# RatInABox-Lab/RatInABox

Measured on AMD Instinct MI355X. Metric: agent-steps/sec (whole node) at 4096 agents x 1024 PlaceCells, higher is better.
Workload: dtype f32 rates / f64 motion

## Files before the change

### include/riab_hip.h

```cpp
#ifndef RIAB_HIP_H
#define RIAB_HIP_H

#include <stdint.h>

#ifdef __cplusplus
extern "C" {
#endif

#define RIAB_ABI_VERSION 11
#define RIAB_MAX_WALLS 64
#define RIAB_MAX_TEST_ANGLES 360
#define RIAB_STATE_ROWS 12
#define RIAB_HIST_ROWS 8
#define RIAB_MAX_BOUNCES 16

enum {
  RIAB_OK = 0,
  RIAB_EINVAL = -1,
  RIAB_EALIGN = -2,
  RIAB_ETOOBIG = -3,
  RIAB_EUNSUPPORTED = -4,
  RIAB_EFULL = -5,
  RIAB_EPARTIAL = -6,
  RIAB_ECHANGED = -7
// ... 318 lines not shown
  RIAB_TW_EP_START = 4,
  RIAB_TW_EP_ANY_ENDED = 5,
  RIAB_TW_STARTED = 6,
  RIAB_TW_TERMINAL = 7,
  RIAB_TW_GOAL_LIST = 8,
  RIAB_TW_ROWS = 24
};
int riab_task_world_step(const RiabEnv* env, const RiabTask* task, double* task_state, double* world,
                         const double* pos_x, const double* pos_y, int64_t B, double t_env, double* reward_out,
                         uint8_t* terminal_out, uint64_t* met_scratch, int32_t* cand_scratch, int32_t* ctl,
                         int32_t* diag, riab_stream_t stream);
int riab_task_world_reset(const RiabEnv* env, const RiabTask* task, double* task_state, double* world, int64_t B,
                          int64_t agent_id0, double t_env, int32_t n_select, int32_t ordered, uint64_t seed,
                          uint64_t counter, int32_t teleport, const double* new_x, const double* new_y,
                          double* pos_x, double* pos_y, float* hist_x, float* hist_y, double* ep_log,
                          int64_t ep_log_cap, int32_t* ep_count, int32_t only_if_terminal, double gv_scale,
                          double* gv_x, double* gv_y, int32_t* diag, riab_stream_t stream);
int riab_task_world_goal_vector(const RiabEnv* env, const RiabTask* task, double* task_state, const double* world,
                                const double* pos_x, const double* pos_y, int64_t B, double scale, double* out_x,
                                double* out_y, riab_stream_t stream);

int riab_plan_set_task(RiabPlan* plan, const RiabTask* task, double* task_state, int64_t task_B, double t_env,
                       double dt_env, double* reward_out, uint8_t* terminal_out, int32_t* task_diag,
                       int32_t auto_reset, int32_t n_select, int32_t ordered, uint64_t task_seed,
                       uint64_t reset_counter, int32_t teleport, double* ep_log, int64_t ep_log_cap,
                       int32_t* ep_count, double scripted_speed);
double riab_plan_task_clock(const RiabPlan* plan);
int riab_plan_set_task_world(RiabPlan* plan, double* world, uint64_t* met_scratch, int32_t* cand_scratch, int32_t* ctl);

enum { RIAB_CTRL_STARTED = 0, RIAB_CTRL_TIMEOUTS = 1, RIAB_CTRL_ABORT = 2, RIAB_CTRL_SERIALISED = 3,
       RIAB_CTRL_STAMPS = 8,
       RIAB_CTRL_TRAJ_STAMPS = 12,
       RIAB_CTRL_PROGRESS = 32 };
#define RIAB_CTRL_PROGRESS_WORD(w) (RIAB_CTRL_PROGRESS + 32 * ((w) >> 2) + ((w) & 3))
#define RIAB_CTRL_WORDS(B) (RIAB_CTRL_PROGRESS + 32 * (((B) + 255) / 256))
enum { RIAB_TIMING_STAMPS = 0, RIAB_TIMING_EVENTS = 1 };
typedef struct RiabSimulate {
  const RiabEnv* env;
  const RiabMotion* motion;
  double* state;
  int64_t B;
  int64_t agent_id0;
  const double* drift;
  const double* noise;
  const double* forced_pos;
  const double* resample_pos;
  uint64_t seed;
  uint64_t step0;
  int32_t T;
  int32_t n_pops;
  const struct RiabPopulation* pops;
  float* hist;
  int32_t* diag;
  uint32_t* ctrl;
  int32_t timed_pop;
  int32_t timing_mode;
  const struct RiabWatch* watch;
  int32_t n_watch;
} RiabSimulate;
typedef struct RiabWatch {
  const void* live;
  const void* snapshot;
  int64_t bytes;
} RiabWatch;
typedef struct RiabStreamer RiabStreamer;
RiabStreamer* riab_streamer_create(void);
void riab_streamer_destroy(RiabStreamer* h);
enum { RIAB_STREAMER_OPT_GATE = 0, RIAB_STREAMER_OPT_POLL_MAX = 1, RIAB_STREAMER_OPT_HEAD_ROWS = 2,
       RIAB_STREAMER_OPT_SIDE_STREAM = 3, RIAB_STREAMER_OPT_STEP_NS = 4, RIAB_STREAMER_OPT_LEAD_MBPS = 5,
       RIAB_STREAMER_OPT_STRICT = 6, RIAB_STREAMER_OPT_SPIN_LIMIT = 7 };
enum { RIAB_GATE_ALWAYS = 0, RIAB_GATE_WHEN_BUSY = 1, RIAB_GATE_RESERVED = 2 };
int riab_streamer_configure(RiabStreamer* h, int32_t option, int32_t value);
int riab_streamer_warmup(RiabStreamer* h, riab_stream_t stream);
int riab_simulate(RiabStreamer* h, const RiabSimulate* run, riab_stream_t stream);
int riab_watch_compare(const RiabWatch* watch, int32_t n);
float riab_streamer_last_rate_ms(RiabStreamer* h);
enum { RIAB_FORM_NONE = 0, RIAB_FORM_ONE_KERNEL = 1, RIAB_FORM_CHUNKS = 2, RIAB_FORM_SERIAL = 3, RIAB_FORM_POPULATIONS = 4,
       RIAB_FORM_HEAD_AND_PIECES = 5 };
int riab_streamer_last_form(RiabStreamer* h);
int64_t riab_streamer_info(RiabStreamer* h, int32_t which);

enum { RIAB_OPT_TRAJ_KERNEL = 0, RIAB_OPT_FUSED_TASK = 1, RIAB_OPT_BVC_BOX = 2, RIAB_OPT_NT_STORES = 3,
       RIAB_OPT_PUB_SINGLE_ROWS = 4, RIAB_OPT_POLL_SLEEP = 5, RIAB_OPT_FUSED_STEP = 6, RIAB_OPT_STEP1_SPIN = 7,
       RIAB_OPT_STEP1_RESIDENCY = 8, RIAB_OPT_COUNT = 9 };
int riab_set_option(int32_t option, int32_t value);

int riab_host_wait_spin(int32_t on);

typedef struct RiabTDParams {
  float dt;
  float tau;
  float tau_e;
  float eta;
  float L2;
  int64_t B;
  int64_t Bp;
  int32_t n;
  int32_t Mp;
} RiabTDParams;

typedef struct RiabTDLayer {
  const float* rates;
  float* trace;
  float* wt;
  int32_t n_in;
} RiabTDLayer;

int riab_td_forward_tail(const RiabTDParams* p, const RiabTDLayer* layers, int32_t n_layers, const float* v,
                         float* v_last, float* dvdt, int32_t with_trace, riab_stream_t stream);

int64_t riab_td_workspace(const RiabTDParams* p, const RiabTDLayer* layers, int32_t n_layers);

int riab_td_update(const RiabTDParams* p, const RiabTDLayer* layers, int32_t n_layers, const void* reward,
                   int32_t reward_f64, int64_t reward_ld_n, int64_t reward_ld_b, const float* v, const float* dvdt,
                   const float* prime, float* td, int32_t fuse_trace, float* workspace, int64_t workspace_floats,
                   riab_stream_t stream);

int riab_td_reset(const RiabTDParams* p, const RiabTDLayer* layers, int32_t n_layers, float* const* rows,
                  int32_t n_rows, const uint8_t* mask, riab_stream_t stream);

int riab_td_learn_step(const RiabTDParams* p, const RiabTDLayer* layers, int32_t n_layers, const void* reward,
                       int32_t reward_f64, int64_t reward_ld_n, int64_t reward_ld_b, float* v, float* v_last, float* dvdt,
                       const float* prime, float* td, const uint8_t* mask, int32_t zero_v, float* workspace,
                       int64_t workspace_floats, riab_stream_t stream);

enum {
  RIAB_REWARD_NONE = 0,
  RIAB_REWARD_TASK = 1,
  RIAB_REWARD_POINTER = 2,
  RIAB_REWARD_POPULATION = 3
};
int riab_plan_set_learner(RiabPlan* plan, int32_t index, const RiabTDParams* p, float* const* traces, float* v_last,
                          float* dvdt, float* td, float* workspace, int64_t workspace_floats, int32_t reward_kind,
                          const void* reward, int32_t reward_f64, int64_t reward_ld_n, int64_t reward_ld_b,
                          int32_t reward_index);

enum {
  RIAB_THETA_NONE = 0,
  RIAB_THETA_BEHIND = 1,
  RIAB_THETA_AHEAD = 2
};
enum {
  RIAB_THETA_DIAG_BEHIND = 0,
  RIAB_THETA_DIAG_AHEAD = 1,
  RIAB_THETA_DIAG_ROLLOUT = 2,
  RIAB_THETA_DIAG_FAR = 3
};

int riab_theta_sequence_step(const RiabEnv* env, const double* lead_state, int64_t B, int64_t n_agents, double* ring,
                             int32_t capacity, int32_t lookback, int64_t n_records, int32_t branch, double phase, double d_half,
                             double theta_frac, const double* future, const int32_t* count, int32_t K, double* pos_out,
                             int32_t* diag, riab_stream_t stream);

int riab_theta_sequence_rollout(const RiabEnv* env, const RiabMotion* motion, const double* lead_state,
                                double* forward_state, int64_t B, int64_t n_agents, int64_t agent_id0, const double* z_in,
                                double* z_out,
                                uint64_t seed, uint64_t step0, int32_t K, double forward_distance, double* future,
                                int32_t* count, int32_t* motion_diag, int32_t* diag, riab_stream_t stream);

int riab_shift_agent_position(const double* lead_state, int64_t B, double shift_m, double* pos_out, riab_stream_t stream);

enum {
  RIAB_DUMB_DIAG_WALL_CUTS = 0,
  RIAB_DUMB_DIAG_BOUNDARY = 1,
  RIAB_DUMB_DIAG_SATURATIONS = 2
};

// ... 66 lines not shown
```

### ratinabox_amd/_lib.py

```python
import ctypes as C
import os

import torch

from . import _build

ABI_VERSION = 11
MAX_WALLS = 64
STATE_ROWS = 12
HIST_ROWS = 8

S_POS_X, S_POS_Y, S_VEL_X, S_VEL_Y, S_ROT_VEL, S_MVEL_X, S_MVEL_Y, S_MROT_VEL, S_HD_X, S_HD_Y, S_DIST, S_DWALL = range(12)
H_POS_X, H_POS_Y, H_VEL_X, H_VEL_Y, H_HD_X, H_HD_Y, H_ROT_VEL, H_DIST = range(8)

PC_DESCRIPTIONS = {"gaussian": 0, "gaussian_threshold": 1, "diff_of_gaussians": 2, "one_hot": 3, "top_hat": 4}
GEOMETRIES = {"euclidean": 0, "line_of_sight": 1, "geodesic": 2}
GC_DESCRIPTIONS = {"rectified_cosines": 0, "shifted_cosines": 1}


class RiabEnv(C.Structure):
    _fields_ = [("extent", C.c_double * 4), ("scale", C.c_double), ("periodic", C.c_int32),
                ("n_walls", C.c_int32), ("walls", C.c_void_p), ("polygon", C.c_int32), ("n_boundary", C.c_int32),
                ("hole_mask", C.c_uint64)]

# ... 235 lines not shown
    "riab_probe_compute_units": (C.c_int, [C.c_void_p, C.c_void_p]),
    "riab_plan_info": (C.c_int64, [C.c_void_p, C.c_int32]),
    "riab_task_step": (C.c_int, [C.POINTER(RiabEnv), C.POINTER(RiabTask), C.c_void_p, C.c_void_p, C.c_void_p, C.c_int64,
                                 C.c_double, C.c_void_p, C.c_void_p, C.c_void_p, C.c_void_p]),
    "riab_task_goal_vector": (C.c_int, [C.POINTER(RiabEnv), C.POINTER(RiabTask), C.c_void_p, C.c_void_p, C.c_void_p, C.c_int64,
                                        C.c_double, C.c_void_p, C.c_void_p, C.c_void_p]),
    "riab_plan_set_task": (C.c_int, [C.c_void_p, C.POINTER(RiabTask), C.c_void_p, C.c_int64, C.c_double, C.c_double,
                                     C.c_void_p, C.c_void_p, C.c_void_p, C.c_int32, C.c_int32, C.c_int32, C.c_uint64,
                                     C.c_uint64, C.c_int32, C.c_void_p, C.c_int64, C.c_void_p, C.c_double]),
    "riab_plan_task_clock": (C.c_double, [C.c_void_p]),
    "riab_task_reset": (C.c_int, [C.POINTER(RiabEnv), C.POINTER(RiabTask), C.c_void_p, C.c_void_p, C.c_int64, C.c_int64,
                                  C.c_double, C.c_int32, C.c_int32, C.c_uint64, C.c_uint64, C.c_int32, C.c_void_p,
                                  C.c_void_p, C.c_void_p, C.c_void_p, C.c_void_p, C.c_void_p, C.c_void_p, C.c_int64,
                                  C.c_void_p, C.c_void_p, C.c_void_p]),
    "riab_task_world_step": (C.c_int, [C.POINTER(RiabEnv), C.POINTER(RiabTask), C.c_void_p, C.c_void_p, C.c_void_p, C.c_void_p,
                                       C.c_int64, C.c_double, C.c_void_p, C.c_void_p, C.c_void_p, C.c_void_p, C.c_void_p,
                                       C.c_void_p, C.c_void_p]),
    "riab_task_world_reset": (C.c_int, [C.POINTER(RiabEnv), C.POINTER(RiabTask), C.c_void_p, C.c_void_p, C.c_int64, C.c_int64,
                                        C.c_double, C.c_int32, C.c_int32, C.c_uint64, C.c_uint64, C.c_int32, C.c_void_p,
                                        C.c_void_p, C.c_void_p, C.c_void_p, C.c_void_p, C.c_void_p, C.c_void_p, C.c_int64,
                                        C.c_void_p, C.c_int32, C.c_double, C.c_void_p, C.c_void_p, C.c_void_p, C.c_void_p]),
    "riab_plan_set_task_world": (C.c_int, [C.c_void_p, C.c_void_p, C.c_void_p, C.c_void_p, C.c_void_p]),
    "riab_task_world_goal_vector": (C.c_int, [C.POINTER(RiabEnv), C.POINTER(RiabTask), C.c_void_p, C.c_void_p, C.c_void_p,
                                              C.c_void_p, C.c_int64, C.c_double, C.c_void_p, C.c_void_p, C.c_void_p]),
    "riab_streamer_create": (C.c_void_p, []),
    "riab_streamer_destroy": (None, [C.c_void_p]),
    "riab_simulate": (C.c_int, [C.c_void_p, C.POINTER(RiabSimulate), C.c_void_p]),
    "riab_streamer_warmup": (C.c_int, [C.c_void_p, C.c_void_p]),
    "riab_watch_compare": (C.c_int, [C.c_void_p, C.c_int32]),
    "riab_streamer_configure": (C.c_int, [C.c_void_p, C.c_int32, C.c_int32]),
    "riab_streamer_last_rate_ms": (C.c_float, [C.c_void_p]),
    "riab_streamer_last_form": (C.c_int, [C.c_void_p]),
    "riab_streamer_info": (C.c_int64, [C.c_void_p, C.c_int32]),
    "riab_host_wait_spin": (C.c_int, [C.c_int32]),
    "riab_set_option": (C.c_int, [C.c_int32, C.c_int32]),
    "riab_abi_sizeof": (C.c_int64, [C.c_int32]),
    "riab_abi_version": (C.c_int, []),
    "riab_strerror": (C.c_char_p, [C.c_int]),
}


class RiabError(RuntimeError):
    pass


def _load():
    path = _build.LIB_PATH
    override = os.environ.get("RIAB_HIP_LIB")
    if override:
        path = override
    elif _build.is_stale():
        try:
            path = _build.build()
        except Exception as e:
            if not os.path.exists(path):
                raise ImportError(
                    "ratinabox_amd: libriab_hip.so is missing and could not be built with hipcc "
                    f"({e}). There is no CPU fallback; build it with `python -m ratinabox_amd._build`.") from e
            import warnings
            warnings.warn(f"ratinabox_amd: libriab_hip.so is older than its sources and could not be rebuilt ({e}); "
                          "loading the existing library", RuntimeWarning)
    lib = C.CDLL(path)
    for name, (res, args) in PROTOTYPES.items():
        fn = getattr(lib, name)
        fn.restype = res
        fn.argtypes = args
    if lib.riab_abi_version() != ABI_VERSION:
        raise ImportError(f"libriab_hip.so ABI {lib.riab_abi_version()} != binding ABI {ABI_VERSION}: rebuild")
    mirrors = ((0, RiabEnv), (1, RiabMotion), (2, RiabRateIO), (3, RiabPopulation), (4, RiabTask), (5, RiabFFInput),
               (7, RiabSimulate), (8, RiabWatch), (9, RiabTDParams), (10, RiabTDLayer), (11, RiabMLPLayer))
    for which, cls in mirrors:
        if lib.riab_abi_sizeof(which) != C.sizeof(cls):
            raise ImportError(f"libriab_hip.so: sizeof({cls.__name__}) is {lib.riab_abi_sizeof(which)} in the library, "
                              f"{C.sizeof(cls)} in the binding: rebuild (python -m ratinabox_amd._build --force)")
    if lib.riab_abi_sizeof(6) != TS_ROWS:
        raise ImportError(f"libriab_hip.so: RIAB_TS_ROWS is {lib.riab_abi_sizeof(6)}, the binding has {TS_ROWS}: rebuild")
    return lib, path


lib, LIB_PATH = _load()


OPTIONS = {"traj_kernel": 0, "fused_task": 1, "bvc_box": 2, "nt_stores": 3, "pub_single_rows": 4, "poll_sleep": 5,
           "fused_step": 6, "step1_spin": 7, "step1_residency": 8}


def set_option(name, value):
    old = lib.riab_set_option(OPTIONS[name], int(value))
    if old < 0:
        raise RiabError(f"riab_set_option({name}, {value}) refused")
    return old


for _name, _opt, _val in (("RIAB_NO_PC", "traj_kernel", 1), ("RIAB_TRAJ2", "traj_kernel", 2), ("RIAB_NO_FUSED_TASK", "fused_task", 0),
                          ("RIAB_NO_BVC_BOX", "bvc_box", 0), ("RIAB_NT_STORES_WIDE", "nt_stores", 1),
                          ("RIAB_NO_FUSED_STEP", "fused_step", 0), ("RIAB_FUSED_STEP_PLAIN_STORES", "fused_step", 2)):
    if os.environ.get(_name):
        set_option(_opt, _val)
for _name, _opt in (("RIAB_PUB_SINGLE_ROWS", "pub_single_rows"), ("RIAB_POLL_SLEEP", "poll_sleep"),
                    ("RIAB_STEP1_SPIN", "step1_spin"), ("RIAB_STEP1_RESIDENCY", "step1_residency")):
    if os.environ.get(_name):
        set_option(_opt, int(os.environ[_name]))


def strerror(code):
    return lib.riab_strerror(int(code)).decode()


def check(code, what):
    if code != 0:
        raise RiabError(f"{what} failed with code {code}: {strerror(code)}")


_ENV_DATA = getattr(os.environ, "_data", None)


def env(name, default=None):
    if _ENV_DATA is not None:
        v = _ENV_DATA.get(name.encode() if os.name != "nt" else name.upper())
        return default if v is None else (v.decode() if isinstance(v, bytes) else v)
    return os.environ.get(name, default)


def ptr(t):
    return None if t is None else C.c_void_p(t.data_ptr())


def current_stream():
    import torch
    raw = getattr(torch._C, "_cuda_getCurrentRawStream", None)
    if raw is not None:
        return C.c_void_p(raw(torch.cuda.current_device()))
    return C.c_void_p(torch.cuda.current_stream().cuda_stream)


_COMPUTE_UNITS = {}


def compute_units(device_index):
    n = _COMPUTE_UNITS.get(device_index)
    if n is None:
        import torch
        forced = os.environ.get("RIAB_COMPUTE_UNITS")
        if forced:
            n = int(forced)
        else:
            with torch.cuda.device(device_index):
                scratch = torch.zeros(CU_PROBE_WORDS, dtype=torch.int32, device=f"cuda:{device_index}")
                check(lib.riab_probe_compute_units(ptr(scratch), current_stream()), "riab_probe_compute_units")
                n = int(scratch[CU_PROBE_WORDS - 1].item())
            props = torch.cuda.get_device_properties(device_index).multi_processor_count
            if n < 1 or n > props:
                n = props
        _COMPUTE_UNITS[device_index] = n
    return n
```

### ratinabox_amd/csrc/riab_rates.hip

```cpp
#include <hip/hip_ext.h>

#include <type_traits>

#include "riab_device.h"
#include "riab_rate_cells.h"
#include "riab_handover.h"
#include "riab_launch.h"
#ifndef RIAB_SPIKE_POLICY_GATED
#define RIAB_SPIKE_POLICY_GATED RIAB_STORE_NT
#endif
#ifndef RIAB_SPIKE_POLICY_WIDE
#define RIAB_SPIKE_POLICY_WIDE RIAB_STORE_NT
#endif

namespace riab {


template <class Cell, int SPK, int CPB, bool NT>
__global__ __launch_bounds__(256) void rate_kernel_wide(const RateArgs a, Cell cell) {
  __shared__ double s_lds[Cell::LDS_DOUBLES];
  cell.stage(s_lds);
  constexpr int NP = Cell::NP;
  const int lane = threadIdx.x & 63;
  const int c0 = blockIdx.y * CPB;
  const uint32_t t = blockIdx.z;
  const uint32_t q = blockIdx.x * 256u + threadIdx.x;
  const bool live = q < (uint32_t)a.qrow;
  const uint32_t qc = live ? q : 0u;
  const int pi = c0 * NP + lane;
  const float mine = (lane < NP * CPB && pi < a.n * NP) ? cell.tab[pi] : 0.0f;
  const typename Cell::Pos P = cell.load(a, (int64_t)t * a.pos_ld + 4 * (int64_t)qc);
  int64_t off = ((int64_t)t * a.n + c0) * a.B + 4 * (int64_t)qc;
  const uint32_t step = a.step0 + t;
  const uint32_t group = a.group0 + qc;
  const SpikeCtx k = a.spike_ctx();
  RIAB_CELL_GROUP(Cell, CPB, cell, mine, P, c0, a.n, a.fr_scale, a.fr_min, a.rates, off, a.B, live,
                  NT ? RIAB_STORE_WT : RIAB_STORE_PLAIN, SPK == 1, SPK == 2, NT ? RIAB_STORE_WT : RIAB_SPIKE_POLICY_WIDE, k, step, group)
}

template <class Cell, int SPK>
__global__ __launch_bounds__(256) void rate_kernel_generic(const RateArgs a, Cell cell) {
  __shared__ double s_lds[Cell::LDS_DOUBLES];
  cell.stage(s_lds);
  constexpr int NP = Cell::NP;
  const uint32_t p4 = blockIdx.x * 256u + threadIdx.x;
  const bool live = p4 < a.nquads;
  const uint32_t pc = live ? p4 : 0u;
  const uint32_t t = pc / (uint32_t)a.qrow;
  const uint32_t q = pc - t * (uint32_t)a.qrow;
  const typename Cell::Pos P = cell.load(a, (int64_t)t * a.pos_ld + 4 * (int64_t)q);
  const int c0 = blockIdx.y * a.cells_per_block;
  const int c1 = min(a.n, c0 + a.cells_per_block);
  int64_t off = ((int64_t)t * a.n + c0) * a.B + 4 * (int64_t)q;
  const uint32_t step = a.step0 + t;
  const uint32_t group = a.group0 + q;
  const int lane = threadIdx.x & 63;
  for (int cb = c0; cb < c1; cb += 64) {
    float mine[NP];
    const int cm = min(cb + lane, a.n - 1);
#pragma unroll
    for (int i = 0; i < NP; ++i) mine[i] = cell.tab[cm * NP + i];
    const int cnt = min(64, c1 - cb);
    for (int j = 0; j < cnt; ++j) {
      float p[NP];
#pragma unroll
      for (int i = 0; i < NP; ++i)
        p[i] = __builtin_bit_cast(float, __builtin_amdgcn_readlane(__builtin_bit_cast(int, mine[i]), j));
      v4f r = cell.eval(p, P);
      r = finish_rate(post_scale(cell, p, P, r * a.fr_scale + a.fr_min), P);
      if (live) {
        store_stream<RIAB_STORE_NT>(a.rates + off, r);
        if (SPK == 1) spike_store<false>(a.spike_ctx(), r, off, step, (uint32_t)(cb + j), group);
        if (SPK == 2) spike_store<true>(a.spike_ctx(), r, off, step, (uint32_t)(cb + j), group);
      }
      off += a.B;
    }
  }
}

template <int GX>
__global__ __launch_bounds__(256) void place_one_hot_kernel(const RateArgs a, PlaceCell<RIAB_PC_GAUSSIAN, GX> cell) {
  __shared__ double s_lds[PlaceCell<RIAB_PC_GAUSSIAN, GX>::LDS_DOUBLES];
  cell.stage(s_lds);
  const uint32_t p4 = blockIdx.x * 256u + threadIdx.x;
  if (p4 >= a.nquads) return;
  const uint32_t t = p4 / (uint32_t)a.qrow;
  const uint32_t q = p4 - t * (uint32_t)a.qrow;
  const PosQuad P = cell.load(a, (int64_t)t * a.pos_ld + 4 * (int64_t)q);
  float best[4] = {INFINITY, INFINITY, INFINITY, INFINITY};
  int arg[4] = {0, 0, 0, 0};
// ... 86 lines not shown
    off += a.B;
  }
}

__global__ __launch_bounds__(256) void noise_kernel(float* noise, float* rates, const float* z_in, int n,
                                                    int64_t qrow, int T, float theta_dt, float sigma_dt, uint32_t k0,
                                                    uint32_t k1, uint32_t step0, uint32_t tag, uint32_t group0) {
  const int64_t q = (int64_t)blockIdx.x * 256 + threadIdx.x;
  if (q >= qrow) return;
  const int64_t row = (int64_t)n * qrow * 4;
  for (int c = blockIdx.y; c < n; c += gridDim.y) {
    const int64_t off = ((int64_t)c * qrow + q) * 4;
    v4f x = ldv4(noise + off);
    for (int t = 0; t < T; ++t) {
      v4f z;
      if (z_in) {
        z = ldv4(z_in + t * row + off);
      } else {
        const u32x4 w = philox4x32_spikes(step0 + (uint32_t)t, (uint32_t)c, group0 + (uint32_t)q, tag, k0, k1);
        const float u0 = ((float)(w.x >> 8) + 0.5f) * 0x1.0p-24f, u1 = (float)(w.y >> 8) * 0x1.0p-24f;
        const float u2 = ((float)(w.z >> 8) + 0.5f) * 0x1.0p-24f, u3 = (float)(w.w >> 8) * 0x1.0p-24f;
        const float r0 = sqrtf(-2.0f * logf(u0)), r1 = sqrtf(-2.0f * logf(u2));
        z = v4f{r0 * __builtin_amdgcn_cosf(u1), r0 * __builtin_amdgcn_sinf(u1), r1 * __builtin_amdgcn_cosf(u3),
                r1 * __builtin_amdgcn_sinf(u3)};
      }
      x = x + (-theta_dt) * x + sigma_dt * z;
      const v4f r = ldv4(rates + t * row + off);
      *reinterpret_cast<v4f*>(rates + t * row + off) = r + x;
    }
    *reinterpret_cast<v4f*>(noise + off) = x;
  }
}

__global__ __launch_bounds__(256) void fill_kernel(float* dst, int64_t n4, float value) {
  const int64_t i = (int64_t)blockIdx.x * 256 + threadIdx.x;
  if (i < n4) reinterpret_cast<v4f*>(dst)[i] = v4f{value, value, value, value};
}

struct StreamArgs {
  uint32_t* ctrl;
  uint32_t step_base;
  uint32_t spin_limit;
  uint32_t stamps;
  uint32_t sleep_max;
  uint32_t serial_rows;
  uint32_t serial_gap;
};
__device__ __forceinline__ bool ended_just_now(const uint32_t* ctrl, uint32_t gap_ticks) {
  const unsigned long long end = ld_agent(reinterpret_cast<const uint64_t*>(ctrl + RIAB_CTRL_TRAJ_STAMPS + 2));
  const unsigned long long now = __builtin_amdgcn_s_memrealtime();
  return now >= end && now - end < (unsigned long long)gap_ticks;
}
__device__ __forceinline__ int stream_progress(const StreamArgs& s, uint32_t q, int lane) {
  int rel = 0x7fffffff;
  if (lane < 4) {
    const uint32_t v = ld_agent(s.ctrl + RIAB_CTRL_PROGRESS + 32 * q + lane);
    rel = (int)(v - s.step_base);
    rel = rel < 0 ? 0 : rel;
  }
  const int r0 = __builtin_amdgcn_readlane(rel, 0), r1 = __builtin_amdgcn_readlane(rel, 1);
  const int r2 = __builtin_amdgcn_readlane(rel, 2), r3 = __builtin_amdgcn_readlane(rel, 3);
  return __builtin_amdgcn_readfirstlane(min(min(r0, r1), min(r2, r3)));
}
__device__ __forceinline__ void stream_wait(const StreamArgs& s, uint32_t q, int t, int lane) {
  int known = stream_progress(s, q, lane);
  for (uint32_t spins = 0; known <= t; ++spins) {
    const uint32_t ab = ld_agent(s.ctrl + RIAB_CTRL_ABORT);
    if (__builtin_amdgcn_readfirstlane((int)ab)) return;
    if (spins >= s.spin_limit) {
      if (lane == 0) {
        atomicAdd(s.ctrl + RIAB_CTRL_TIMEOUTS, 1u);
        st_agent(s.ctrl + RIAB_CTRL_ABORT, 1u);
      }
      return;
    }
    if (spins < 4) __builtin_amdgcn_s_sleep(4);
    else if (spins < 16 || s.sleep_max <= 16) __builtin_amdgcn_s_sleep(16);
    else if (s.sleep_max >= 48) __builtin_amdgcn_s_sleep(48);
    else __builtin_amdgcn_s_sleep(32);
    known = stream_progress(s, q, lane);
  }
}

template <class Cell, int SPK, int CPB, bool LONG, int WAVES>
__global__ __launch_bounds__(64 * WAVES) void rate_kernel_gated(const RateArgs a, Cell cell, const StreamArgs s) {
  __shared__ double s_lds[Cell::LDS_DOUBLES];
  cell.stage(s_lds);
  constexpr int NP = Cell::NP;
  static_assert(WAVES % 4 == 0, "four waves share a (1024 agents) x (CPB cells) tile");
  const int lane = threadIdx.x & 63;
  const int wv = __builtin_amdgcn_readfirstlane((int)(threadIdx.x >> 6));
  const int c0 = (int)(blockIdx.y * (WAVES / 4) + (wv >> 2)) * CPB;
  const uint32_t t = blockIdx.z;
  const uint32_t q = blockIdx.x * 256u + (threadIdx.x & 255u);
  const uint32_t wq = (uint32_t)__builtin_amdgcn_readfirstlane((int)(blockIdx.x * 4u + (uint32_t)(wv & 3)));
  if (wq * 64u >= (uint32_t)a.qrow || c0 >= a.n) return;
  const int pi = c0 * NP + lane;
  const float mine = (lane < NP * CPB && pi < a.n * NP) ? cell.tab[pi] : 0.0f;
  const bool grid_first = t == 0 && blockIdx.x == 0 && blockIdx.y == 0 && wv == 0;
  if (s.stamps && grid_first && lane == 0)
    st_agent(reinterpret_cast<uint64_t*>(s.ctrl + RIAB_CTRL_STAMPS), (uint64_t)__builtin_amdgcn_s_memrealtime());
  if (s.serial_rows >= 8u && grid_first) {
    if (stream_progress(s, wq, lane) >= (int)s.serial_rows && ended_just_now(s.ctrl, s.serial_gap) && lane == 0)
      atomicAdd(s.ctrl + RIAB_CTRL_SERIALISED, 1u);
  }
#ifdef RIAB_PIPE_PROFILE
  riab_g64* const dbg = (riab_g64*)(uintptr_t)(s.ctrl + 2048);
  const bool first_wg = blockIdx.x == 0 && blockIdx.y == 0 && threadIdx.x == 0;
  if (first_wg) dbg[1 * 64 + t] = (unsigned long long)__builtin_amdgcn_s_memrealtime();
#endif
  stream_wait(s, wq, (int)t, lane);
#ifdef RIAB_PIPE_PROFILE
  if (first_wg) dbg[2 * 64 + t] = (unsigned long long)__builtin_amdgcn_s_memrealtime();
#endif
  const int64_t po = (int64_t)t * a.pos_ld + 4 * (int64_t)q;
  const typename Cell::Pos P = cell.load_agent(a, po);
  int64_t off = ((int64_t)t * a.n + c0) * a.B + 4 * (int64_t)q;
  const uint32_t step = a.step0 + t;
  const uint32_t group = a.group0 + q;
  const SpikeCtx k = a.spike_ctx();
  RIAB_CELL_GROUP(Cell, CPB, cell, mine, P, c0, a.n, a.fr_scale, a.fr_min, a.rates, off, a.B, true, RIAB_STORE_NT, SPK == 1, false,
                  RIAB_SPIKE_POLICY_GATED, k, step, group)
#ifdef RIAB_PIPE_PROFILE
  if (c0 + CPB >= a.n && blockIdx.x + 1 == gridDim.x && (threadIdx.x & 255u) == 0) {
    drain_stores();
    dbg[3 * 64 + t] = (unsigned long long)__builtin_amdgcn_s_memrealtime();
  }
#endif
  if (s.stamps && t + 1 == gridDim.z && c0 + CPB >= a.n) {
    drain_stores();
    if (lane == 0) fetch_max_agent(reinterpret_cast<uint64_t*>(s.ctrl + RIAB_CTRL_STAMPS + 2), (uint64_t)__builtin_amdgcn_s_memrealtime());
  }
}

__global__ __launch_bounds__(64) void stream_gate_kernel(uint32_t* ctrl, uint32_t started_target, uint32_t n_traj,
                                                         uint32_t progress_target, uint32_t spin_limit, uint32_t sleep_long,
                                                         uint32_t final_target, uint32_t serial_gap) {
  const int lane = threadIdx.x;
  for (uint32_t spins = 0;; ++spins) {
    const uint32_t v = ld_agent(ctrl + RIAB_CTRL_STARTED);
    bool ok = (int32_t)(v - started_target) >= 0;
    bool all_done = ok && final_target != 0u && spins == 0u;
    if (ok) {
      for (uint32_t w = lane; w < n_traj; w += 64) {
        const uint32_t p = ld_agent(ctrl + RIAB_CTRL_PROGRESS_WORD(w));
        ok = ok && (int32_t)(p - progress_target) >= 0;
        all_done = all_done && (int32_t)(p - final_target) >= 0;
      }
    }
    if (spins == 0u && final_target != 0u && n_traj > 0u && __builtin_amdgcn_ballot_w64(!all_done) == 0 &&
        ended_just_now(ctrl, serial_gap) && lane == 0)
      atomicAdd(ctrl + RIAB_CTRL_SERIALISED, 1u);
    if (__builtin_amdgcn_ballot_w64(!ok) == 0) return;
    if (ld_agent(ctrl + RIAB_CTRL_ABORT)) return;
    if (spins >= spin_limit) {
      if (lane == 0) {
        atomicAdd(ctrl + RIAB_CTRL_TIMEOUTS, 1u);
        st_agent(ctrl + RIAB_CTRL_ABORT, 1u);
      }
      return;
    }
    if (sleep_long && spins >= 64) __builtin_amdgcn_s_sleep(127);
    else if (sleep_long) __builtin_amdgcn_s_sleep(8);
    else __builtin_amdgcn_s_sleep(16);
  }
}

__global__ __launch_bounds__(64) void stream_open_kernel(uint32_t* ctrl, uint32_t n_traj, uint32_t step_base) {
  for (uint32_t w = threadIdx.x; w < n_traj; w += 64)
    st_agent(ctrl + RIAB_CTRL_PROGRESS_WORD(w), step_base);
  if (threadIdx.x == 0)
    st_agent(ctrl + RIAB_CTRL_STARTED, 0u);
}

static int check_io(const RiabRateIO* io, int n, bool need_pos, bool need_hd) {
  if (!io || n <= 0 || io->T <= 0 || io->B <= 0 || !io->rates) return RIAB_EINVAL;
  if (need_pos && (!io->pos_x || !io->pos_y)) return RIAB_EINVAL;
  if (need_hd && (!io->hd_x || !io->hd_y)) return RIAB_EINVAL;
  if (io->B % 4 != 0 || io->pos_ld % 4 != 0 || io->agent_id0 % 4 != 0) return RIAB_EALIGN;
  const uintptr_t m = (uintptr_t)io->rates | (uintptr_t)io->pos_x | (uintptr_t)io->pos_y | (uintptr_t)io->hd_x |
                      (uintptr_t)io->hd_y | (uintptr_t)io->u_in;
  if (m & 15) return RIAB_EALIGN;
  if ((uintptr_t)io->spikes & 3) return RIAB_EALIGN;
  if (io->u_in && !io->spikes) return RIAB_EINVAL;
  if (io->T * (io->B / 4) >= ((int64_t)1 << 31)) return RIAB_ETOOBIG;
  return RIAB_OK;
}

static RateArgs make_args(const RiabRateIO* io, int n) {
  RateArgs a;
  a.pos_x = io->pos_x;
  a.pos_y = io->pos_y;
  a.hd_x = io->hd_x;
  a.hd_y = io->hd_y;
  a.pos_ld = io->pos_ld;
  a.qrow = io->B / 4;
  a.nquads = io->T * a.qrow;
  a.B = io->B;
  a.rates = io->rates;
  a.spikes = io->spikes;
  a.u_in = io->u_in;
  a.dt = io->dt;
  a.fr_scale = io->max_fr - io->min_fr;
  a.fr_min = io->min_fr;
  a.k0 = (uint32_t)io->seed;
  a.k1 = (uint32_t)(io->seed >> 32);
  a.step0 = (uint32_t)io->step0;
// ... 41 lines not shown
  if (geometry == RIAB_GEOM_EUCLIDEAN) return RIAB_OK;
  if (env->n_walls - 4 > RIAB_MAX_WALLS) return RIAB_ETOOBIG;
  if (geometry == RIAB_GEOM_GEODESIC && env->n_walls > 5) return RIAB_EUNSUPPORTED;
  return RIAB_OK;
}
static int place_geometry_check(const RiabEnv* env, int geometry) {
  if (!env->periodic && geometry != RIAB_GEOM_EUCLIDEAN && env->n_walls > 4 && !env->walls) return RIAB_EINVAL;
  return place_geometry_refused(env, geometry);
}
template <class F>
static int visit_place_geometry(const RiabEnv* env, int geometry, F&& f) {
  if (env->periodic) return f(std::integral_constant<int, 3>{});
  switch (geometry) {
    case RIAB_GEOM_EUCLIDEAN: return f(std::integral_constant<int, 0>{});
    case RIAB_GEOM_LINE_OF_SIGHT: return f(std::integral_constant<int, 1>{});
    case RIAB_GEOM_GEODESIC: return f(std::integral_constant<int, 2>{});
    default: return RIAB_EINVAL;
  }
}
template <int GX>
static int internal_walls(const RiabEnv* env) {
  const int n_internal = env->n_walls > 4 ? env->n_walls - 4 : 0;
  return (GX == 2 && n_internal > 1) ? 1 : n_internal;
}
template <int GX>
static PlaceCell<RIAB_PC_GAUSSIAN, GX> make_place_cell(const RiabEnv* env, const float* table, float top_hat_width, int n_internal) {
  return place_cell<RIAB_PC_GAUSSIAN, GX>(table, (float)env->scale, (float)(env->scale / 2), top_hat_width * top_hat_width,
                                          env->walls, n_internal, make_env_shape(env));
}
template <int GX, class F>
static int visit_place_desc(int desc, const PlaceCell<RIAB_PC_GAUSSIAN, GX>& base, int otherwise, F&& f) {
  switch (desc) {
    case RIAB_PC_GAUSSIAN: return f(base);
    case RIAB_PC_GAUSSIAN_THRESHOLD: return f(base.template as<RIAB_PC_GAUSSIAN_THRESHOLD>());
    case RIAB_PC_DIFF_OF_GAUSSIANS: return f(base.template as<RIAB_PC_DIFF_OF_GAUSSIANS>());
    case RIAB_PC_TOP_HAT: return f(base.template as<RIAB_PC_TOP_HAT>());
    default: return otherwise;
  }
}
template <class F>
static int visit_grid_desc(int desc, const float* table, float f0, F&& f) {
  if (desc == RIAB_GC_RECTIFIED) return f(GridCell<RIAB_GC_RECTIFIED>{table, f0, 1.0f / (1.0f - f0)});
  if (desc == RIAB_GC_SHIFTED) return f(GridCell<RIAB_GC_SHIFTED>{table, f0, 1.0f});
  return RIAB_EINVAL;
}

template <int GX>
static int launch_place(const RiabRateIO* io, int n, int desc, const PlaceCell<RIAB_PC_GAUSSIAN, GX>& base,
                        hipStream_t s) {
  if (desc == RIAB_PC_ONE_HOT) {
    RateArgs a = make_args(io, n);
    dim3 grid = generic_grid(&a);
    grid.y = 1;
    hipLaunchKernelGGL((place_one_hot_kernel<GX>), grid, dim3(256), 0, s, a, base);
    return (int)hipGetLastError();
  }
  return visit_place_desc(desc, base, RIAB_EINVAL, [&](const auto& c) { return launch_rate(io, n, c, s); });
}

static uint32_t serial_gap_ticks() {
  static uint32_t ticks = 0;
  if (!ticks) {
    int dev = 0, khz = 0;
    if (hipGetDevice(&dev) != hipSuccess || hipDeviceGetAttribute(&khz, hipDeviceAttributeWallClockRate, dev) != hipSuccess || khz <= 0)
      khz = 100000;
    ticks = (uint32_t)((long long)khz * 25 / 1000);
  }
  return ticks;
}

struct StreamLaunch {
  StreamArgs st;
  hipEvent_t ev0, ev1;
  int T;
  bool spikes;
  bool reserve;
  bool dry_run;
  hipStream_t s;
};

template <class Cell>
static int launch_stream_cell(const RateArgs& a, const Cell& cell, const StreamLaunch& L) {
  constexpr int CPB = (Cell::NP * 2 * Cell::CPB <= 64) ? 2 * Cell::CPB : Cell::CPB;
  using Kernel = void (*)(const RateArgs, Cell, const StreamArgs);
  static constexpr Kernel kGated[8] = {
      rate_kernel_gated<Cell, 0, CPB, false, 4>,  rate_kernel_gated<Cell, 0, CPB, true, 4>,
      rate_kernel_gated<Cell, 1, CPB, false, 4>,  rate_kernel_gated<Cell, 1, CPB, true, 4>,
      rate_kernel_gated<Cell, 0, CPB, false, 12>, rate_kernel_gated<Cell, 0, CPB, true, 12>,
      rate_kernel_gated<Cell, 1, CPB, false, 12>, rate_kernel_gated<Cell, 1, CPB, true, 12>};
  const int T = L.T;
  const int64_t groups = (a.n + CPB - 1) / CPB;
  if (T > 65535 || groups > 65535) return RIAB_ETOOBIG;
  const bool reserve = L.reserve;
  const int variant = (reserve ? 4 : 0) + (L.spikes ? 2 : 0) + (T > 256 ? 1 : 0);
  if (reserve) {
    static int regs[8] = {0, 0, 0, 0, 0, 0, 0, 0};
    int& r = regs[variant];
    if (r == 0) {
      hipFuncAttributes attr;
      const void* f = (const void*)kGated[variant];
      r = (hipFuncGetAttributes(&attr, f) == hipSuccess && attr.numRegs > 0) ? attr.numRegs : 1 << 20;
      if (r < (1 << 20) && 2 * (int64_t)attr.sharedSizeBytes + 81920 > 160 * 1024) r = 1 << 20;
      (void)hipGetLastError();
    }
    if (6 * ((r + 7) / 8 * 8) + traj_kernel_regs() > 512) return RIAB_EUNSUPPORTED;
  }
  if (L.dry_run) return RIAB_OK;
  static bool launched[8] = {false, false, false, false, false, false, false, false};
  bool& seen = launched[variant];
  StreamArgs st = L.st;
  if (!seen) st.serial_rows = 0u;
  seen = true;
  const dim3 grid((unsigned)((a.qrow + 255) / 256), (unsigned)(reserve ? (groups + 2) / 3 : groups), (unsigned)T);
  const dim3 block(reserve ? 768 : 256);
  if (L.ev0 || L.ev1) hipExtLaunchKernelGGL(kGated[variant], grid, block, 0, L.s, L.ev0, L.ev1, 0u, a, cell, st);
  else hipLaunchKernelGGL(kGated[variant], grid, block, 0, L.s, a, cell, st);
  return (int)hipGetLastError();
}

template <class F>
static int visit_stream_cell(const RiabEnv* env, const RiabPopulation* pop, F&& f) {
  switch (pop->kind) {
    case RIAB_POP_PLACE:
      return visit_place_geometry(env, pop->geometry, [&](auto gx) {
        return visit_place_desc(pop->description, make_place_cell<decltype(gx)::value>(env, pop->table, pop->top_hat_width, internal_walls<decltype(gx)::value>(env)),
                                RIAB_EUNSUPPORTED, f);
      });
    case RIAB_POP_GRID: return visit_grid_desc(pop->description, pop->table, pop->f0, f);
    case RIAB_POP_HDC: return f(HDCell<0>{pop->table, 0.0f, nullptr, nullptr});
    case RIAB_POP_PLANE_WAVE: return f(PlaneWaveCell{pop->table});
    default: return RIAB_EUNSUPPORTED;
  }
}

int stream_supported(const RiabEnv* env, const RiabPopulation* pop, int64_t B) {
  if (!env || !pop || pop->n <= 0 || B <= 0 || B % 256 != 0) return RIAB_EUNSUPPORTED;
  if (pop->noise_state) return RIAB_EUNSUPPORTED;
  switch (pop->kind) {
    case RIAB_POP_PLACE:
      if (pop->description == RIAB_PC_ONE_HOT) return RIAB_EUNSUPPORTED;
      if (place_geometry_refused(env, pop->geometry)) return RIAB_EUNSUPPORTED;
      return pop->table ? RIAB_OK : RIAB_EINVAL;
    case RIAB_POP_GRID:
    case RIAB_POP_HDC:
    case RIAB_POP_PLANE_WAVE: return pop->table ? RIAB_OK : RIAB_EINVAL;
    default: return RIAB_EUNSUPPORTED;
  }
}

int launch_rate_stream(const RiabEnv* env, const RiabPopulation* pop, const float* hist, int64_t B, int32_t T, float dt,
                       uint64_t seed, uint64_t step0, int64_t agent_id0, uint32_t* ctrl, uint32_t spin_limit, bool stamps,
                       hipStream_t s, hipEvent_t ev_start, hipEvent_t ev_stop, bool dry_run, bool reserve,
                       uint32_t serial_rows) {
  int rc = stream_supported(env, pop, B);
  if (rc) return rc;
  if (!hist || !ctrl || !pop->rates_base || T <= 0 || pop->capacity_rows < T || agent_id0 % 4) return RIAB_EINVAL;
  if ((((uintptr_t)hist | (uintptr_t)pop->rates_base) & 15) || ((uintptr_t)pop->spikes_base & 3)) return RIAB_EALIGN;
  RiabRateIO io = pop->io;
  hist_rows_io(&io, hist, B, (int64_t)RIAB_HIST_ROWS * B);
  io.T = T;
  io.rates = pop->rates_base;
  io.spikes = pop->spikes_base;
  io.u_in = nullptr;
  io.dt = dt;
  io.seed = seed;
  io.step0 = step0 + 1;
  io.agent_id0 = agent_id0;
  const RateArgs a = make_args(&io, pop->n);
  StreamArgs st;
  st.ctrl = ctrl;
  st.step_base = (uint32_t)step0;
  st.spin_limit = spin_limit;
  st.stamps = stamps ? 1u : 0u;
  st.sleep_max = (uint32_t)g_options[RIAB_OPT_POLL_SLEEP];
  st.serial_rows = serial_rows;
  st.serial_gap = serial_gap_ticks();
  const StreamLaunch L{st, ev_start, ev_stop, T, pop->spikes_base != nullptr, reserve, dry_run, s};
  return visit_stream_cell(env, pop, [&](const auto& c) { return launch_stream_cell(a, c, L); });
}

int launch_stream_open(uint32_t* ctrl, uint32_t n_traj, uint32_t step_base, hipStream_t s) {
  hipLaunchKernelGGL(stream_open_kernel, dim3(1), dim3(64), 0, s, ctrl, n_traj, step_base);
  return (int)hipGetLastError();
}

int launch_stream_gate(uint32_t* ctrl, uint32_t started_target, uint32_t n_traj, uint32_t progress_target,
                       uint32_t spin_limit, bool sleep_long, uint32_t final_target, hipStream_t s) {
  static bool launched = false;
  if (!launched) final_target = 0u;
  launched = true;
  hipLaunchKernelGGL(stream_gate_kernel, dim3(1), dim3(64), 0, s, ctrl, started_target, n_traj, progress_target, spin_limit,
// ... 100 lines not shown
  return visit_place_geometry(env, geometry, [&](auto gx) {
    return random_spatial_dispatch<decltype(gx)::value>(env, io, anchors, M, targets, n, (hipStream_t)stream);
  });
}

extern "C" int riab_grid_cells(const RiabRateIO* io, const float* table, int32_t n, int32_t description, float f0,
                               riab_stream_t stream) {
  if (!table) return RIAB_EINVAL;
  const int rc = check_io(io, n, true, false);
  if (rc) return rc;
  return visit_grid_desc(description, table, f0, [&](const auto& c) { return launch_rate(io, n, c, (hipStream_t)stream); });
}

extern "C" int riab_plane_wave_neurons(const RiabRateIO* io, const float* table, int32_t n, riab_stream_t stream) {
  if (!table) return RIAB_EINVAL;
  const int rc = check_io(io, n, true, false);
  if (rc) return rc;
  return launch_rate(io, n, PlaneWaveCell{table}, (hipStream_t)stream);
}

extern "C" int riab_head_direction_cells(const RiabRateIO* io, const float* table, int32_t n,
                                         riab_stream_t stream) {
  if (!table) return RIAB_EINVAL;
  const int rc = check_io(io, n, false, true);
  if (rc) return rc;
  HDCell<0> c{table, 0.0f, nullptr, nullptr};
  return launch_rate(io, n, c, (hipStream_t)stream);
}

extern "C" int riab_velocity_cells(const RiabRateIO* io, const float* table, int32_t n, float one_sigma_speed,
                                   const double* vel_x, const double* vel_y, riab_stream_t stream) {
  if (!table || !(one_sigma_speed > 0.0f) || (vel_x == nullptr) != (vel_y == nullptr)) return RIAB_EINVAL;
  const int rc = check_io(io, n, false, vel_x == nullptr);
  if (rc) return rc;
  if (vel_x && io->T != 1) return RIAB_EINVAL;
  if (((uintptr_t)vel_x | (uintptr_t)vel_y) & 31) return RIAB_EALIGN;
  HDCell<1> c{table, 1.0f / one_sigma_speed, vel_x, vel_y};
  return launch_rate(io, n, c, (hipStream_t)stream);
}

extern "C" int riab_speed_cell(const RiabRateIO* io, float one_sigma_speed, riab_stream_t stream) {
  if (!(one_sigma_speed > 0.0f)) return RIAB_EINVAL;
  const int rc = check_io(io, 1, false, true);
  if (rc) return rc;
  HDCell<2> c{io->hd_x, 1.0f / one_sigma_speed, nullptr, nullptr};
  return launch_rate(io, 1, c, (hipStream_t)stream);
}

extern "C" int riab_spikes(const RiabRateIO* io, int32_t n, riab_stream_t stream) {
  const int rc = check_io(io, n, false, false);
  if (rc) return rc;
  if (!io->spikes) return RIAB_EINVAL;
  RateArgs a = make_args(io, n);
  const dim3 grid = generic_grid(&a);
  if (io->u_in) hipLaunchKernelGGL((spikes_kernel<true>), grid, dim3(256), 0, (hipStream_t)stream, a);
  else hipLaunchKernelGGL((spikes_kernel<false>), grid, dim3(256), 0, (hipStream_t)stream, a);
  return (int)hipGetLastError();
}

extern "C" int riab_neuron_noise(float* noise, float* rates, const float* z_in, int32_t n, int64_t B, int32_t T,
                                 float theta_dt, float sigma_dt, uint64_t seed, uint64_t step, int32_t pop_id,
                                 int64_t agent_id0, riab_stream_t stream) {
  if (!noise || !rates || n <= 0 || B <= 0 || T <= 0) return RIAB_EINVAL;
  if (B % 4 || agent_id0 % 4 || (((uintptr_t)noise | (uintptr_t)rates | (uintptr_t)z_in) & 15)) return RIAB_EALIGN;
  const int64_t qrow = B / 4;
  dim3 grid((unsigned)((qrow + 255) / 256), (unsigned)(n < 65535 ? n : 65535), 1);
  hipLaunchKernelGGL(noise_kernel, grid, dim3(256), 0, (hipStream_t)stream, noise, rates, z_in, n, qrow, T, theta_dt,
                     sigma_dt, (uint32_t)seed, (uint32_t)(seed >> 32), (uint32_t)step,
                     riab::stream_tag(RIAB_TAG_NOISE, pop_id), (uint32_t)(agent_id0 / 4));
  return (int)hipGetLastError();
}

extern "C" int riab_fill(void* dst, int64_t bytes, float value, riab_stream_t stream) {
  if (!dst || bytes <= 0) return RIAB_EINVAL;
  if ((bytes & 15) || ((uintptr_t)dst & 15)) return RIAB_EALIGN;
  const int64_t n4 = bytes / 16;
  const int64_t blocks = (n4 + 255) / 256;
  if (blocks > 0x7fffffffLL) return RIAB_ETOOBIG;
  hipLaunchKernelGGL(fill_kernel, dim3((unsigned)blocks), dim3(256), 0, (hipStream_t)stream, (float*)dst, n4, value);
  return (int)hipGetLastError();
}

namespace riab {
int g_options[RIAB_OPT_COUNT] = {0, 1, 1, 0, 4, 48, 1, 22, 1};
}
extern "C" int riab_set_option(int32_t option, int32_t value) {
  static const int lo[RIAB_OPT_COUNT] = {0, 0, 0, 0, 0, 1, 0, 0, 0};
  static const int hi[RIAB_OPT_COUNT] = {2, 1, 1, 1, 64, 127, 2, 30, 1};
  if (option < 0 || option >= RIAB_OPT_COUNT || value < lo[option] || value > hi[option]) return RIAB_EINVAL;
  const int old = riab::g_options[option];
  riab::g_options[option] = value;
  return old;
}

extern "C" int riab_abi_version(void) { return RIAB_ABI_VERSION; }

extern "C" const char* riab_strerror(int code) {
  switch (code) {
    case RIAB_OK: return "ok";
    case RIAB_EINVAL: return "invalid argument (null pointer, non-positive size or unknown enum)";
    case RIAB_EALIGN: return "agent axis not a multiple of 4 or row pointer not 16-byte aligned";
    case RIAB_ETOOBIG: return "too many walls / test angles / objects for the LDS staging (vector cells: 768 bytes per object, 213 objects in 160 KiB)";
    case RIAB_EUNSUPPORTED: return "combination not supported on device";
    case RIAB_EFULL: return "a step plan's history chunk is full: attach a new chunk";
    case RIAB_EPARTIAL: return "a launch failed after the trajectory kernel had been launched: the state has advanced, the rates of this call are incomplete";
    case RIAB_ECHANGED: return "a watched host array differs from its snapshot: the cached device tables are stale (nothing was launched)";
    default: return code > 0 ? hipGetErrorString((hipError_t)code) : "unknown riab error";
  }
}
```

Before: 1.415 billion.

## Add row-wise store map for gated rate kernel with LDS-shared agent positions

Adds a ROWS variant of the gated streaming rate kernel. The four waves of a tile share agent positions through LDS, and each wave computes and stores whole cell rows (CPB/4 cells across 256 agents) instead of every wave handling all cells for its own 64 agents. The aim is longer contiguous store streams per cell row and fewer per-wave parameter reads. It costs an LDS staging buffer and a __syncthreads, and it is used only for non-spiking populations with simple Pos, by default when T > 256.

```diff
diff --git a/include/riab_hip.h b/include/riab_hip.h
--- a/include/riab_hip.h
+++ b/include/riab_hip.h
@@ -424,7 +424,7 @@
 
 enum { RIAB_OPT_TRAJ_KERNEL = 0, RIAB_OPT_FUSED_TASK = 1, RIAB_OPT_BVC_BOX = 2, RIAB_OPT_NT_STORES = 3,
        RIAB_OPT_PUB_SINGLE_ROWS = 4, RIAB_OPT_POLL_SLEEP = 5, RIAB_OPT_FUSED_STEP = 6, RIAB_OPT_STEP1_SPIN = 7,
-       RIAB_OPT_STEP1_RESIDENCY = 8, RIAB_OPT_COUNT = 9 };
+       RIAB_OPT_STEP1_RESIDENCY = 8, RIAB_OPT_RATE_ROWS = 9, RIAB_OPT_COUNT = 10 };
 int riab_set_option(int32_t option, int32_t value);
 
 int riab_host_wait_spin(int32_t on);
diff --git a/ratinabox_amd/_lib.py b/ratinabox_amd/_lib.py
--- a/ratinabox_amd/_lib.py
+++ b/ratinabox_amd/_lib.py
@@ -341,7 +341,7 @@
 
 
 OPTIONS = {"traj_kernel": 0, "fused_task": 1, "bvc_box": 2, "nt_stores": 3, "pub_single_rows": 4, "poll_sleep": 5,
-           "fused_step": 6, "step1_spin": 7, "step1_residency": 8}
+           "fused_step": 6, "step1_spin": 7, "step1_residency": 8, "rate_rows": 9}
 
 
 def set_option(name, value):
@@ -357,7 +357,8 @@
     if os.environ.get(_name):
         set_option(_opt, _val)
 for _name, _opt in (("RIAB_PUB_SINGLE_ROWS", "pub_single_rows"), ("RIAB_POLL_SLEEP", "poll_sleep"),
-                    ("RIAB_STEP1_SPIN", "step1_spin"), ("RIAB_STEP1_RESIDENCY", "step1_residency")):
+                    ("RIAB_STEP1_SPIN", "step1_spin"), ("RIAB_STEP1_RESIDENCY", "step1_residency"),
+                    ("RIAB_RATE_ROWS", "rate_rows")):
     if os.environ.get(_name):
         set_option(_opt, int(os.environ[_name]))
 
diff --git a/ratinabox_amd/csrc/riab_rate_tile_map.h b/ratinabox_amd/csrc/riab_rate_tile_map.h
--- /dev/null
+++ b/ratinabox_amd/csrc/riab_rate_tile_map.h
@@ -0,0 +1,22 @@
+#pragma once
+#if defined(__HIPCC__) || defined(__CUDACC__)
+#define RIAB_TILE_FN __host__ __device__ inline constexpr
+#else
+#define RIAB_TILE_FN inline constexpr
+#endif
+
+namespace riab {
+
+RIAB_TILE_FN int rate_tile_stride(bool pure) { return pure ? 2 : 1; }
+RIAB_TILE_FN int rate_tile_first(bool pure, int cpb, int tiles, int y, int g) {
+  return pure ? 2 * cpb * (tiles * (y >> 1) + g) + (y & 1) : cpb * (tiles * y + g);
+}
+RIAB_TILE_FN int rate_tile_grid_y(bool pure, int cpb, int tiles, int n) {
+  return pure ? 2 * (((n + 2 * cpb - 1) / (2 * cpb) + tiles - 1) / tiles) : ((n + cpb - 1) / cpb + tiles - 1) / tiles;
+}
+RIAB_TILE_FN int rate_tile_span(bool pure, int cpb) { return pure ? 2 * cpb - 1 : cpb; }
+
+RIAB_TILE_FN int rate_store_cell(bool rows, int cpb, int w, int i) { return rows ? w * (cpb / 4) + (i >> 2) : i; }
+RIAB_TILE_FN int rate_store_quad(bool rows, int w, int i, int lane) { return rows ? 64 * (i & 3) + lane : 64 * w + lane; }
+
+}
diff --git a/ratinabox_amd/csrc/riab_rates.hip b/ratinabox_amd/csrc/riab_rates.hip
--- a/ratinabox_amd/csrc/riab_rates.hip
+++ b/ratinabox_amd/csrc/riab_rates.hip
@@ -6,6 +6,7 @@
 #include "riab_rate_cells.h"
 #include "riab_handover.h"
 #include "riab_launch.h"
+#include "riab_rate_tile_map.h"
 #ifndef RIAB_SPIKE_POLICY_GATED
 #define RIAB_SPIKE_POLICY_GATED RIAB_STORE_NT
 #endif
@@ -258,21 +259,25 @@
   }
 }
 
-template <class Cell, int SPK, int CPB, bool LONG, int WAVES>
+template <class Cell, int SPK, int CPB, bool LONG, int WAVES, bool ROWS>
 __global__ __launch_bounds__(64 * WAVES) void rate_kernel_gated(const RateArgs a, Cell cell, const StreamArgs s) {
   __shared__ double s_lds[Cell::LDS_DOUBLES];
   cell.stage(s_lds);
   constexpr int NP = Cell::NP;
   static_assert(WAVES % 4 == 0, "four waves share a (1024 agents) x (CPB cells) tile");
+  static_assert(!ROWS || CPB % 4 == 0, "a wave takes whole cells of the tile");
+  static_assert(!ROWS || SPK == 0, "populations that draw spikes keep the column map (launch_stream_cell)");
   const int lane = threadIdx.x & 63;
   const int wv = __builtin_amdgcn_readfirstlane((int)(threadIdx.x >> 6));
-  const int c0 = (int)(blockIdx.y * (WAVES / 4) + (wv >> 2)) * CPB;
+  const int c0 = rate_tile_first(false, CPB, WAVES / 4, (int)blockIdx.y, wv >> 2);
   const uint32_t t = blockIdx.z;
   const uint32_t q = blockIdx.x * 256u + (threadIdx.x & 255u);
   const uint32_t wq = (uint32_t)__builtin_amdgcn_readfirstlane((int)(blockIdx.x * 4u + (uint32_t)(wv & 3)));
-  if (wq * 64u >= (uint32_t)a.qrow || c0 >= a.n) return;
-  const int pi = c0 * NP + lane;
-  const float mine = (lane < NP * CPB && pi < a.n * NP) ? cell.tab[pi] : 0.0f;
+  const bool wave_live = wq * 64u < (uint32_t)a.qrow && c0 < a.n;
+  if (!ROWS && !wave_live) return;
+  const int cw0 = ROWS ? c0 + rate_store_cell(true, CPB, wv & 3, 0) : c0;
+  const int pi = cw0 * NP + lane;
+  const float mine = (lane < NP * (ROWS ? CPB / 4 : CPB) && pi < a.n * NP) ? cell.tab[pi] : 0.0f;
   const bool grid_first = t == 0 && blockIdx.x == 0 && blockIdx.y == 0 && wv == 0;
   if (s.stamps && grid_first && lane == 0)
     st_agent(reinterpret_cast<uint64_t*>(s.ctrl + RIAB_CTRL_STAMPS), (uint64_t)__builtin_amdgcn_s_memrealtime());
@@ -285,20 +290,49 @@
   const bool first_wg = blockIdx.x == 0 && blockIdx.y == 0 && threadIdx.x == 0;
   if (first_wg) dbg[1 * 64 + t] = (unsigned long long)__builtin_amdgcn_s_memrealtime();
 #endif
-  stream_wait(s, wq, (int)t, lane);
+  if (wave_live) stream_wait(s, wq, (int)t, lane);
 #ifdef RIAB_PIPE_PROFILE
   if (first_wg) dbg[2 * 64 + t] = (unsigned long long)__builtin_amdgcn_s_memrealtime();
 #endif
   const int64_t po = (int64_t)t * a.pos_ld + 4 * (int64_t)q;
-  const typename Cell::Pos P = cell.load_agent(a, po);
-  int64_t off = ((int64_t)t * a.n + c0) * a.B + 4 * (int64_t)q;
   const uint32_t step = a.step0 + t;
-  const uint32_t group = a.group0 + q;
   const SpikeCtx k = a.spike_ctx();
-  RIAB_CELL_GROUP(Cell, CPB, cell, mine, P, c0, a.n, a.fr_scale, a.fr_min, a.rates, off, a.B, true, RIAB_STORE_NT, SPK == 1, false,
-                  RIAB_SPIKE_POLICY_GATED, k, step, group)
+  if constexpr (!ROWS) {
+    const typename Cell::Pos P = cell.load_agent(a, po);
+    int64_t off = ((int64_t)t * a.n + c0) * a.B + 4 * (int64_t)q;
+    const uint32_t group = a.group0 + q;
+    RIAB_CELL_GROUP(Cell, CPB, cell, mine, P, c0, a.n, a.fr_scale, a.fr_min, a.rates, off, a.B, true, RIAB_STORE_NT, SPK == 1, false,
+                    RIAB_SPIKE_POLICY_GATED, k, step, group)
+  } else {
+    __shared__ typename Cell::Pos s_pos[(WAVES / 4) * 256];
+    typename Cell::Pos* const sp = s_pos + (wv >> 2) * 256;
+    const int w = wv & 3;
+    if (wave_live) sp[64 * w + lane] = cell.load_agent(a, po);
+    __syncthreads();
+    if (c0 >= a.n) return;
+    const uint32_t q0 = blockIdx.x * 256u;
+    const int64_t row0 = ((int64_t)t * a.n + c0) * a.B;
+    typename Cell::Pos P[4];
+#pragma unroll
+    for (int i = 0; i < 4; ++i) P[i] = sp[64 * i + lane];
+#pragma unroll
+    for (int i = 0; i < CPB; ++i) {
+      const int j = rate_store_cell(true, CPB, w, i);
+      const uint32_t qi = q0 + (uint32_t)rate_store_quad(true, w, i, lane);
+      if (c0 + j < a.n && (q0 + 64u * (uint32_t)(i & 3)) < (uint32_t)a.qrow) {
+        float p_[NP];
+#pragma unroll
+        for (int i_ = 0; i_ < NP; ++i_)
+          p_[i_] = __builtin_bit_cast(float, __builtin_amdgcn_readlane(__builtin_bit_cast(int, mine), (i >> 2) * NP + i_));
+        v4f r_ = cell.eval(p_, P[i & 3]);
+        r_ = finish_rate(post_scale(cell, p_, P[i & 3], r_ * a.fr_scale + a.fr_min), P[i & 3]);
+        const int64_t off = row0 + (int64_t)j * a.B + 4 * (int64_t)qi;
+        store_stream<RIAB_STORE_NT>(a.rates + off, r_);
+      }
+    }
+  }
 #ifdef RIAB_PIPE_PROFILE
-  if (c0 + CPB >= a.n && blockIdx.x + 1 == gridDim.x && (threadIdx.x & 255u) == 0) {
+  if (c0 + CPB >= a.n && blockIdx.x + 1 == gridDim.x && (threadIdx.x & 255u) == (ROWS ? 192u : 0u)) {
     drain_stores();
     dbg[3 * 64 + t] = (unsigned long long)__builtin_amdgcn_s_memrealtime();
   }
@@ -506,19 +540,26 @@
 template <class Cell>
 static int launch_stream_cell(const RateArgs& a, const Cell& cell, const StreamLaunch& L) {
   constexpr int CPB = (Cell::NP * 2 * Cell::CPB <= 64) ? 2 * Cell::CPB : Cell::CPB;
+  constexpr bool R = sizeof(typename Cell::Pos) == sizeof(PosQuad) && Cell::LDS_DOUBLES == 1;
   using Kernel = void (*)(const RateArgs, Cell, const StreamArgs);
-  static constexpr Kernel kGated[8] = {
-      rate_kernel_gated<Cell, 0, CPB, false, 4>,  rate_kernel_gated<Cell, 0, CPB, true, 4>,
-      rate_kernel_gated<Cell, 1, CPB, false, 4>,  rate_kernel_gated<Cell, 1, CPB, true, 4>,
-      rate_kernel_gated<Cell, 0, CPB, false, 12>, rate_kernel_gated<Cell, 0, CPB, true, 12>,
-      rate_kernel_gated<Cell, 1, CPB, false, 12>, rate_kernel_gated<Cell, 1, CPB, true, 12>};
+  static constexpr Kernel kGated[16] = {
+      rate_kernel_gated<Cell, 0, CPB, false, 4, false>,  rate_kernel_gated<Cell, 0, CPB, true, 4, false>,
+      rate_kernel_gated<Cell, 1, CPB, false, 4, false>,  rate_kernel_gated<Cell, 1, CPB, true, 4, false>,
+      rate_kernel_gated<Cell, 0, CPB, false, 12, false>, rate_kernel_gated<Cell, 0, CPB, true, 12, false>,
+      rate_kernel_gated<Cell, 1, CPB, false, 12, false>, rate_kernel_gated<Cell, 1, CPB, true, 12, false>,
+      rate_kernel_gated<Cell, 0, CPB, false, 4, R>,      rate_kernel_gated<Cell, 0, CPB, true, 4, R>,
+      rate_kernel_gated<Cell, 1, CPB, false, 4, false>,  rate_kernel_gated<Cell, 1, CPB, true, 4, false>,
+      rate_kernel_gated<Cell, 0, CPB, false, 12, R>,     rate_kernel_gated<Cell, 0, CPB, true, 12, R>,
+      rate_kernel_gated<Cell, 1, CPB, false, 12, false>, rate_kernel_gated<Cell, 1, CPB, true, 12, false>};
   const int T = L.T;
   const int64_t groups = (a.n + CPB - 1) / CPB;
   if (T > 65535 || groups > 65535) return RIAB_ETOOBIG;
   const bool reserve = L.reserve;
-  const int variant = (reserve ? 4 : 0) + (L.spikes ? 2 : 0) + (T > 256 ? 1 : 0);
+  const int opt_rows = g_options[RIAB_OPT_RATE_ROWS];
+  const bool rows = R && !L.spikes && (opt_rows == 2 || (opt_rows == 1 && T > 256));
+  const int variant = (rows ? 8 : 0) + (reserve ? 4 : 0) + (L.spikes ? 2 : 0) + (T > 256 ? 1 : 0);
   if (reserve) {
-    static int regs[8] = {0, 0, 0, 0, 0, 0, 0, 0};
+    static int regs[16] = {0, 0, 0, 0, 0, 0, 0, 0, 0, 0, 0, 0, 0, 0, 0, 0};
     int& r = regs[variant];
     if (r == 0) {
       hipFuncAttributes attr;
@@ -530,7 +571,8 @@
     if (6 * ((r + 7) / 8 * 8) + traj_kernel_regs() > 512) return RIAB_EUNSUPPORTED;
   }
   if (L.dry_run) return RIAB_OK;
-  static bool launched[8] = {false, false, false, false, false, false, false, false};
+  static bool launched[16] = {false, false, false, false, false, false, false, false,
+                              false, false, false, false, false, false, false, false};
   bool& seen = launched[variant];
   StreamArgs st = L.st;
   if (!seen) st.serial_rows = 0u;
@@ -797,11 +839,11 @@
 }
 
 namespace riab {
-int g_options[RIAB_OPT_COUNT] = {0, 1, 1, 0, 4, 48, 1, 22, 1};
+int g_options[RIAB_OPT_COUNT] = {0, 1, 1, 0, 4, 48, 1, 22, 1, 1};
 }
 extern "C" int riab_set_option(int32_t option, int32_t value) {
-  static const int lo[RIAB_OPT_COUNT] = {0, 0, 0, 0, 0, 1, 0, 0, 0};
-  static const int hi[RIAB_OPT_COUNT] = {2, 1, 1, 1, 64, 127, 2, 30, 1};
+  static const int lo[RIAB_OPT_COUNT] = {0, 0, 0, 0, 0, 1, 0, 0, 0, 0};
+  static const int hi[RIAB_OPT_COUNT] = {2, 1, 1, 1, 64, 127, 2, 30, 1, 2};
   if (option < 0 || option >= RIAB_OPT_COUNT || value < lo[option] || value > hi[option]) return RIAB_EINVAL;
   const int old = riab::g_options[option];
   riab::g_options[option] = value;
```

New measurement: 1.310 billion. 0.926x the previous value.
